# joesharratt1229/DT4Image_Restoration

Measured on AMD Instinct MI355X. Metric: pnp_admm_iterations_per_sec, higher is better.
Workload: dtype f32

## Files before the change

### dt4image_restoration_amd/_lib.py

```python
from __future__ import annotations

import ctypes as C
import os

_HERE = os.path.dirname(os.path.abspath(__file__))
LIB_PATH = os.environ.get("PNP_LIB_PATH") or os.path.join(_HERE, "csrc", "libpnpadmm.so")

PNP_FLAG_PROFILE = 1
PNP_FLAG_NO_DENOISER = 2
PNP_FLAG_KEEP_STAGES = 4
PNP_FLAG_BF16_CONVS = 8
PNP_FLAG_PROFILE_LAYERS = 16
PNP_SSIM_CLAMP_X = 1
PNP_RES_COLS = 6
PNP_RES_DELTA = 1
PNP_RES_DC = 2
RESIDUAL_COLUMNS = ("primal", "dx", "dz", "du", "delta", "dc")
PNP_MC_MAX_COILS = 32
PNP_MC_MAX_CG = 64
PNP_CC_MAX_COILS = 64
PNP_PW_MAX_COILS = 64
PNP_ESPIRIT_MAX_COILS = 16
PNP_ESPIRIT_MAX_KSIZE = 8
PNP_ESPIRIT_MAX_N = 512
# ... 78 lines not shown
    "pnp_restore": (C.c_int, [C.c_void_p, _vp, _fp, _fp, _fp, _fp, _vp]),
    "pnp_unet_read_stage": (C.c_int, [C.c_void_p, C.c_int, _fp, C.POINTER(C.c_int), C.POINTER(C.c_int),
                                      C.POINTER(C.c_int), _vp]),
    "pnp_profile_reset": (C.c_int, [C.c_void_p]),
    "pnp_profile_collect": (C.c_int, [C.c_void_p, C.POINTER(C.c_double), C.POINTER(C.c_int64)]),
    "pnp_profile_layers": (C.c_int, [C.c_void_p, C.POINTER(C.c_double), C.POINTER(C.c_int64)]),
    "pnp_conv_algorithms": (C.c_int, [C.c_void_p, C.POINTER(C.c_int32)]),
    "pnp_conv_schedules": (C.c_int, [C.c_void_p, C.POINTER(C.c_int32)]),
    "pnp_bf16_weight_terms": (C.c_int, [C.c_void_p]),
    "pnp_workspace_bytes": (C.c_size_t, [C.c_void_p]),
}

SIGNATURES_NCSENSE = {
    "pnp_nufft_forward_mc": (C.c_int, [C.c_void_p, _fp, _fp, C.c_int, C.c_int, C.c_int, _fp, _vp]),
    "pnp_nufft_adjoint_mc": (C.c_int, [C.c_void_p, _fp, _fp, _fp, C.c_int, C.c_int, C.c_int, _fp, _vp]),
    "pnp_set_kspace_ncsense": (C.c_int, [C.c_void_p, _fp, _fp, C.c_int, C.c_int, _fp, C.c_int, _vp]),
    "pnp_reset_ncsense": (C.c_int, [C.c_void_p, _fp, _fp, _fp, C.c_int, C.c_int, _fp, C.c_int, _fp, _fp, _fp, _vp]),
    "pnp_ncsense_coils": (C.c_int, [C.c_void_p]),
    "pnp_ncsense_cg_residual": (C.c_int, [C.c_void_p, _fp, _vp]),
    "pnp_ncsense_normal": (C.c_int, [C.c_void_p, _fp, _fp, _fp, _vp]),
    "pnp_acquire_ncsense": (C.c_int, [C.c_void_p, _fp, _fp, C.c_int, C.c_int, _fp, C.c_double, C.c_uint64, C.c_int, _fp, _fp, _fp, _vp]),
}

_lib = None


class PnPError(RuntimeError):
    pass


def load() -> C.CDLL:
    global _lib
    if _lib is not None:
        return _lib
    if not os.path.exists(LIB_PATH):
        raise PnPError(f"{LIB_PATH} not found: build it with `python -c 'import __graft_entry__ as g; g.build()'` "
                       f"or `make -C {os.path.dirname(LIB_PATH)}`; there is no CPU fallback")
    lib = C.CDLL(LIB_PATH)
    for name, (res, args) in {**SIGNATURES, **SIGNATURES_NCSENSE}.items():
        fn = getattr(lib, name)
        fn.restype = res
        fn.argtypes = args
    _lib = lib
    return lib


def check(rc: int, what: str) -> None:
    if rc != 0:
        msg = load().pnp_last_error()
        raise PnPError(f"{what} failed ({rc}): {msg.decode() if msg else '?'}")
```

### dt4image_restoration_amd/csrc/conv_kernels.hip

```cpp
#include "pnp_internal.h"
#include "conv_staging.h"
#include <cstring>
#include <cstdlib>

namespace pnp {



const LayerSpec kLayers[N_LAYERS] = {
    {2, 32, 3, 0, SRC_SIGMA, 0},    {32, 32, 3, 0, SRC_PLAIN, 0},   {32, 32, 3, 0, SRC_PLAIN, 0},
    {32, 64, 3, 1, SRC_POOL, 0},    {64, 64, 3, 1, SRC_PLAIN, 0},   {64, 64, 3, 1, SRC_PLAIN, 0},
    {64, 128, 3, 2, SRC_POOL, 0},   {128, 128, 3, 2, SRC_PLAIN, 0}, {128, 128, 3, 2, SRC_PLAIN, 0},
    {128, 256, 3, 3, SRC_POOL, 0},  {256, 256, 3, 3, SRC_PLAIN, 0}, {256, 256, 3, 3, SRC_PLAIN, 0},
    {256, 512, 3, 4, SRC_POOL, 0},  {512, 512, 3, 4, SRC_PLAIN, 0}, {512, 512, 3, 4, SRC_PLAIN, 0},
    {768, 256, 3, 3, SRC_UPCAT, 256}, {256, 256, 3, 3, SRC_PLAIN, 0}, {256, 256, 3, 3, SRC_PLAIN, 0},
    {384, 128, 3, 2, SRC_UPCAT, 128}, {128, 128, 3, 2, SRC_PLAIN, 0}, {128, 128, 3, 2, SRC_PLAIN, 0},
    {192, 64, 3, 1, SRC_UPCAT, 64},  {64, 64, 3, 1, SRC_PLAIN, 0},   {64, 64, 3, 1, SRC_PLAIN, 0},
    {96, 32, 3, 0, SRC_UPCAT, 32},   {32, 32, 3, 0, SRC_PLAIN, 0},   {32, 32, 3, 0, SRC_PLAIN, 0},
    {32, 1, 1, 0, SRC_PLAIN, 0},
};

ConvPlan conv3x3_plan(int N, int H, int W, int Cin, int Cout, bool bf16, int src_mode, bool allow_ws) {
    ConvPlan p{};
    p.tw = W >= 32 ? 32 : (W >= 16 ? 16 : 8);
// ... 623 lines not shown

bool conv3x3_pooled_output_ok(const ConvPlan& p) {
    return p.splitk == 1 && p.mt <= 2 && p.nt == 1 && p.wm == 4;
}

size_t conv3x3_partial_floats(const ConvPlan& p, int N, int H, int W, int Cout) {
    return (p.mt <= 2 && p.wn >= 2) ? (size_t)p.splitk * N * H * W * Cout : 0;
}

Tuning tuning_from_env() {
    Tuning t;
    if (const char* v = getenv("PNP_WINO_MIN_CIN")) t.wino_min_cin = atoi(v);
    if (const char* v = getenv("PNP_WINO_MIN_BLOCKS")) t.wino_min_blocks = atol(v);
    t.wino_big = getenv("PNP_WINO_BIG_GROUPS") != nullptr;
    t.wino_small = getenv("PNP_WINO_SMALL_GROUPS") != nullptr;
    t.no_wino = getenv("PNP_NO_WINOGRAD") != nullptr;
    if (const char* v = getenv("PNP_WINO_F4_MIN_CIN")) t.f4_min_cin = atoi(v);
    t.no_f4 = getenv("PNP_NO_WINO_F4") != nullptr;
    t.no_f4_phased = getenv("PNP_NO_WINO_F4_PHASED") != nullptr;
    t.no_f4_fused_last = getenv("PNP_NO_F4_FUSED_LAST") != nullptr;
    t.no_f4_fused_first = getenv("PNP_NO_F4_FUSED_FIRST") != nullptr;
    if (const char* v = getenv("PNP_WINO_F4_MT16")) t.f4_mt16 = atoi(v);
    if (const char* v = getenv("PNP_WINO_F4_CS")) t.f4_cs = atoi(v);
    if (const char* v = getenv("PNP_WINO_F4_ORDER")) t.f4_order = atoi(v) != 0;
    t.bf16_f32_acts = getenv("PNP_BF16_F32_ACTS") != nullptr;
    t.bf16_no_ws = getenv("PNP_BF16_NO_WS") != nullptr;
    t.bf16_w1 = getenv("PNP_BF16_W1") != nullptr;
    t.bf16_no_holdhi = getenv("PNP_BF16_NO_HOLDHI") != nullptr;
    if (const char* v = getenv("PNP_SLICE128_MIN_N")) t.slice128_min_n = atoi(v);
    if (const char* v = getenv("PNP_TV_NAIVE")) t.tv_naive = atoi(v) != 0;
    if (const char* v = getenv("PNP_HAAR_NAIVE")) t.haar_naive = atoi(v) != 0;
    if (const char* v = getenv("PNP_NCSENSE_COIL_BLOCK")) t.ncsense_block = atoi(v);
    if (const char* v = getenv("PNP_NCSENSE_NAIVE")) t.ncsense_naive = atoi(v) != 0 ? 1 : 0;
    return t;
}

hipError_t raise_lds_cap(const void* fn, int bytes, DeviceOnce& once) {
    int dev = 0;
    hipError_t e = hipGetDevice(&dev);
    if (e != hipSuccess) return e;
    const uint64_t bit = 1ull << (dev & 63);
    if (once.mask.load(std::memory_order_relaxed) & bit) return hipSuccess;
    e = hipFuncSetAttribute(fn, hipFuncAttributeMaxDynamicSharedMemorySize, bytes);
    if (e != hipSuccess) return e;
    once.mask.fetch_or(bit, std::memory_order_relaxed);
    return hipSuccess;
// ... 177 lines not shown
```

### dt4image_restoration_amd/csrc/pnp_capi.hip

```cpp
#include "../../include/pnpadmm.h"
#include "../../include/pnpadmm_ncsense.h"
#include "pnp_internal.h"
#include "denoiser_plan.h"
#include "nufft_plan.h"
#include "block_reduce.h"

#include <cmath>
#include <cstdarg>
#include <cstdio>
#include <cstring>
#include <cstdlib>
#include <initializer_list>
#include <new>
#include <string>
#include <vector>

using namespace pnp;

namespace {

thread_local std::string g_err;

int fail(int code, const char* fmt, ...) {
    char buf[512];
// ... 2061 lines not shown
    PNP_API_BEGIN
    if (!e || !algo28) return fail(PNP_ERR_INVALID, "pnp_conv_algorithms: null argument");
    if (e->cfg.flags & PNP_FLAG_NO_DENOISER) return fail(PNP_ERR_STATE, "pnp_conv_algorithms: handle has no denoiser");
    for (int i = 0; i < N_LAYERS; ++i) algo28[i] = e->dplan.family[i];
    return PNP_OK;
    PNP_API_END("pnp_conv_algorithms")
}

int pnp_conv_schedules(pnp_handle e, int32_t* sched28) {
    PNP_API_BEGIN
    if (!e || !sched28) return fail(PNP_ERR_INVALID, "pnp_conv_schedules: null argument");
    if (e->cfg.flags & PNP_FLAG_NO_DENOISER) return fail(PNP_ERR_STATE, "pnp_conv_schedules: handle has no denoiser");
    for (int i = 0; i < N_LAYERS; ++i) {
        const int at = e->dplan.launch_of[i];
        sched28[i] = 0;
        if (at < 0 || e->dplan.family[i] != FAM_WINO4) continue;
        const WinoPlan& w = e->dplan.launch[at].wino;
        sched28[i] = w.cs ? 4 : (w.mt == 16 ? 3 : (w.phased ? 2 : 1));
    }
    return PNP_OK;
    PNP_API_END("pnp_conv_schedules")
}

int pnp_profile_reset(pnp_handle e) {
    PNP_API_BEGIN
    if (!e) return fail(PNP_ERR_INVALID, "null handle");
    e->ev_used = 0;
    memset(e->cls_ms, 0, sizeof e->cls_ms); memset(e->cls_n, 0, sizeof e->cls_n);
    memset(e->layer_ms, 0, sizeof e->layer_ms); memset(e->layer_n, 0, sizeof e->layer_n);
    return PNP_OK;
    PNP_API_END("pnp_profile_reset")
}

int pnp_profile_collect(pnp_handle e, double* total_ms, int64_t* launches) {
    PNP_API_BEGIN
    if (!e) return fail(PNP_ERR_INVALID, "null handle");
    PNP_ON_DEVICE(e);
    for (size_t i = 0; i < e->ev_used; ++i) {
        float ms = 0.f;
        HIP_TRY(hipEventElapsedTime(&ms, e->events[i].a, e->events[i].b));
        const EventPair& p = e->events[i];
        e->cls_ms[p.cls] += ms; e->cls_n[p.cls] += p.count;
        if (p.layer >= 0) { e->layer_ms[p.layer] += ms; e->layer_n[p.layer] += 1; }
    }
    e->ev_used = 0;
    for (int i = 0; i < PNP_PROFILE_CLASSES; ++i) {
// ... 20 lines not shown
```

### dt4image_restoration_amd/csrc/pnp_internal.h

```cpp
#pragma once
#include <hip/hip_runtime.h>
#include <stdint.h>
#include <stddef.h>
#include <atomic>
#include <vector>

namespace pnp {

struct Tuning {
    int wino_min_cin = 32;
    long wino_min_blocks = 192;
    bool wino_big = false;
    bool wino_small = false;
    bool no_wino = false;
    int f4_min_cin = 32;
    bool no_f4 = false;
    bool no_f4_fused_first = false;
    bool no_f4_fused_last = false;
    bool no_f4_phased = false;
    int f4_mt16 = 0;
    bool bf16_no_ws = false;
    bool bf16_f32_acts = false;
    bool bf16_no_holdhi = false;
    bool bf16_w1 = false;
    int f4_cs = 1;
    int f4_order = 1;
    int slice128_min_n = 192;
    bool tv_naive = false;
    bool haar_naive = false;
    int ncsense_block = 0;
    int ncsense_naive = -1;
};
Tuning tuning_from_env();

struct DeviceOnce { std::atomic<uint64_t> mask{0}; };
hipError_t raise_lds_cap(const void* fn, int bytes, DeviceOnce& once);

enum SrcMode : int { SRC_PLAIN = 0, SRC_SIGMA = 1, SRC_POOL = 2, SRC_UPCAT = 3, SRC_FIRST = 4 };

struct LayerSpec {
    int cin, cout, ksize, level, src, cskip;
};
static constexpr int N_LAYERS = 28;
extern const LayerSpec kLayers[N_LAYERS];

struct ConvArgs {
    const float* src0;
    const float* src1;
// ... 31 lines not shown
    int tiles_x, tiles_y;
};
ConvPlan conv3x3_plan(int N, int H, int W, int Cin, int Cout, bool bf16 = false, int src_mode = SRC_PLAIN, bool allow_ws = true);
hipError_t launch_conv3x3_bf16ws(const ConvArgs& a, const ConvPlan& p, int src_mode, hipStream_t s);
size_t conv3x3_partial_floats(const ConvPlan& p, int N, int H, int W, int Cout);
bool conv3x3_pooled_output_ok(const ConvPlan& p);
bool conv3x3_tensor_fits(int N, int H, int W, int Cin, int Cout);
hipError_t launch_conv3x3(const ConvArgs& a, const ConvPlan& p, int src_mode, hipStream_t s);

size_t conv3x3_pack_floats(int cin, int cout);
void pack_conv3x3_weights(const float* oihw, int cin, int cout, int ck, float* dst);
size_t conv3x3_pack_floats_bf16(int cin, int cout, int terms);
void pack_conv3x3_weights_bf16(const float* oihw, int cin, int cout, int ck, int terms, float* dst);

struct WinoPlan {
    bool use;
    int algo;
    int tw, th, bn, wm, wn, ck, tiles_x, tiles_y;
    int stack;
    int mt;
    int phased;
    int cs;
    int order;
};
WinoPlan winograd_plan(int N, int H, int W, int Cin, int Cout, int src_mode, const Tuning& t, int Cskip = 0);
bool upsample_lines_regular(int H);
size_t winograd4_pack_floats(int cin, int cout);
void pack_winograd4_weights(const float* oihw, int cin, int cout, int ck, float* dst);
hipError_t launch_conv3x3_winograd4(const ConvArgs& a, const WinoPlan& p, int src_mode, hipStream_t s);
size_t winograd_pack_floats(int cin, int cout);
void pack_winograd_weights(const float* oihw, int cin, int cout, int ck, float* dst);
hipError_t launch_conv3x3_winograd(const ConvArgs& a, const WinoPlan& p, int src_mode, hipStream_t s);

hipError_t launch_conv_first(const float* ximg, const float2* z, const float2* u, const float* sigma,
                             const float* tact, const float* w, const float* bias, float* dst,
                             int N, int H, int W, hipStream_t s, bool dst_bf16 = false);
hipError_t launch_conv_last(const float* act, const float* ximg, const float2* z, const float2* u,
                            const float* tact, const float* w, const float* bias, float* out,
                            int N, int H, int W, hipStream_t s);
hipError_t launch_nhwc_to_nchw(const float* src, float* dst, int N, int C, int H, int W, hipStream_t s);

struct FftPlan {
    int h, w;
    float2* tw_h;
    float2* tw_w;
};
// ... 195 lines not shown
```

### dt4image_restoration_amd/csrc/winograd4_kernels.hip

```cpp
#include "pnp_internal.h"
#include "conv_staging.h"
#include <type_traits>

namespace pnp {

#ifdef PNP_STAMPS
#define W4_SLOTS 32
#define W4_WGS 1024
#define W4_N 16
__device__ unsigned long long g_w4_stamps[W4_SLOTS * W4_WGS * W4_N];
static int g_w4_slot = 0;
#define W4T() __builtin_amdgcn_s_memtime()
#endif

namespace {
constexpr double kA = 0.75, kB = 1.5;
constexpr float fA = 0.75f, fB = 1.5f, fA2 = 0.5625f, fB2 = 2.25f, fA3 = 0.421875f, fB3 = 3.375f;
constexpr float fK0 = 1.265625f;
constexpr float fK1 = 2.8125f;

__device__ __forceinline__ float4 f4add(float4 a, float4 b) { return make_float4(a.x + b.x, a.y + b.y, a.z + b.z, a.w + b.w); }
typedef float v2f __attribute__((ext_vector_type(2)));
typedef float f32x4 __attribute__((ext_vector_type(4)));

// ... 646 lines not shown
            if constexpr (FIRST) first_patch(c + 1);
            else park(c + 1, SPLIT ? 1 : 0);
        }
    }
#ifdef PNP_STAMPS
    st_loop1 = W4T();
    st_tmp = st_loop1;
#endif

    wino4_epilogue<TW, STK, MT, WN == 1 && MT == 32 && SRC == SRC_PLAIN>(a, acc, n, th, tg, cl, cb, tx0, ty0, STK ? (th == 0 ? live0 : live1) : true, smem);
#ifdef PNP_STAMPS
    {
        const int w = (int)blockIdx.x - (int)(gridDim.x / 2);
        if (tid == 0 && w >= 0 && w < W4_WGS && a.stamp_slot < W4_SLOTS) {
            unsigned long long* o = g_w4_stamps + ((size_t)a.stamp_slot * W4_WGS + w) * W4_N;
            const unsigned long long te = W4T();
            o[0] = 1; o[1] = st_setup - st_t0; o[2] = st_commit; o[3] = st_trans; o[4] = st_mfma; o[5] = st_loop1 - st_loop0;
            o[6] = te - st_tmp; o[7] = 0; o[8] = te - st_loop1; o[9] = te - st_t0; o[10] = (unsigned long long)nchunks;
        }
    }
#endif
}

template <int TW, bool STK>
__global__ __launch_bounds__(512, 2) void conv3x3_wino4p_kernel(const ConvArgs a) {
    constexpr int CK = 16, CKP = 16, PPP = 4, NT_ = 512, S = 4;
    constexpr int TC = TW / 4, TR = 32 / TC;
    constexpr int TH = 4 * TR;
    constexpr int SUBH = STK ? TH / 2 + 2 : 0;
    constexpr int PH = STK ? 2 * SUBH : TH + 2, PW = TW + 2;
    constexpr int NPIX = PH * PW, ITEMS = NPIX * PPP;
    constexpr int NIT = (ITEMS + NT_ - 1) / NT_;
    constexpr int PLSZ = ((NPIX * 4 + 15) / 16) * 16 + 4;
    constexpr int PATCH = 4 * PLSZ;
    constexpr int PF = 12, KEEP = 3;
    constexpr int PLANE = 32 * CKP;
    constexpr unsigned OOB = 0x80000000u;
    static_assert(!STK || TW == 16, "stacked slices: 16-wide tiles");
    static_assert((2 * PATCH + 36 * PLANE) * 4 <= 160 * 1024, "two patch copies + V in one CU's LDS");

    extern __shared__ __attribute__((aligned(16))) float smem[];
    float* const patch = smem;
    float* const V = smem + 2 * PATCH;
#ifdef PNP_STAMPS
    unsigned long long st_t0 = W4T(), st_setup = 0, st_loop0 = 0, st_commit = 0, st_trans = 0, st_mfma = 0, st_loop1 = 0, st_tmp = 0;
#endif
    const int tid = threadIdx.x, lane = tid & 63;
    const int wid = __builtin_amdgcn_readfirstlane(tid >> 6);
    const int grp = wid >> 2, cq = wid & 3;
    const int th = grp;
    const int tg = lane >> 4, cl = lane & 15;

    const int ny = a.Cout / 64;
    const int bid = blockIdx.x;
    const int ntl = a.tilesX * a.tilesY * (STK ? (a.N + 1) / 2 : a.N);
    int cby, bt;
    wino4_decode(bid, ny, ntl, a.order, cby, bt);
    if (bt >= ntl) return;
    const int tx0 = (bt % a.tilesX) * TW;
    bt /= a.tilesX;
    const int ty0 = (bt % a.tilesY) * TH;
    const int n = STK ? 2 * (bt / a.tilesY) : bt / a.tilesY;
    const int nsl = STK ? (n + 1 < a.N ? 2 : 1) : 1;
    const bool live0 = !(a.tact != nullptr && a.tact[n] > 0.5f);
    const bool live1 = STK && nsl == 2 && !(a.tact != nullptr && a.tact[n + 1] > 0.5f);
    if (!live0 && !live1) return;
    const int cb = cby * 4 + cq;
    const int nchunks = a.Cin / CK;
// ... 9 lines not shown
        const int sub = STK ? py / SUBH : 0;
        const int gy = STK ? py % SUBH - 1 : ty0 + py - 1, gx = tx0 + px - 1;
        voff[k] = (idx < ITEMS && sub < nsl && gy >= 0 && gy < a.H && gx >= 0 && gx < a.W)
                      ? (unsigned)((((sub * a.H + gy) * a.W + gx) * a.Cin + part * 4) * 4) : OOB;
    }
    const int ldst = (tid & 3) * PLSZ + (tid >> 2) * 4;
    float4 raw[NIT];
    auto issue = [&](int c) {
        const int soff = c * CK * 4;
#pragma unroll
        for (int k = 0; k < NIT; ++k)
            raw[k] = __builtin_bit_cast(float4, __builtin_amdgcn_raw_buffer_load_b128(rsrc0, voff[k], soff, 0));
    };
    auto park = [&](int c) {
        float* const dst = patch + (c & 1) * PATCH + ldst;
#pragma unroll
        for (int k = 0; k < NIT; ++k)
            if (tid + k * NT_ < ITEMS) *reinterpret_cast<float4*>(&dst[k * (NT_ / PPP) * 4]) = raw[k];
    };

    auto swz = [](int t16, int g) { return g ^ ((4 - (t16 >> 2)) & 3); };
    const int tgi = tid & 255;
    const int hc = tgi & 7, t16 = (tgi >> 3) & 15;
    const int tj = (wid >> 1) & 1;
    const int tq = 16 * grp + t16;
    const int trow = tq / TC;
    const int wrow = STK ? (trow / (TR / 2)) * SUBH + 4 * (trow % (TR / 2)) : 4 * trow;
    const int win = (hc >> 1) * PLSZ + (wrow * PW + 4 * (tq % TC)) * 4 + 2 * (hc & 1);
    const int vout = tq * CKP + 4 * swz(t16, hc >> 1) + 2 * (hc & 1);

    f32x4 acc[36];
#pragma unroll
    for (int k = 0; k < 36; ++k) acc[k] = f32x4{0.f, 0.f, 0.f, 0.f};

    const size_t stream = (size_t)nchunks * 36 * 64 + kW4Tail / S;
    const float4* const bptr = reinterpret_cast<const float4*>(a.wpack) + (size_t)cb * stream + lane;
    float4 bq[PF];
#pragma unroll
    for (int p = 0; p < KEEP; ++p) bq[p] = bptr[p * 64];
    const int aoff = (16 * th + cl) * CKP + 4 * swz(cl, tg);

    constexpr bool PARK_T = !STK;
    issue(0);
    park(0);
    if constexpr (!PARK_T) { if (grp == 1 && nchunks > 1) { issue(1); park(1); } }
#ifdef PNP_STAMPS
    st_setup = W4T();
    st_loop0 = st_setup;
#endif
    if (grp == 1) __syncthreads();
    for (int c = 0; c < nchunks; ++c) {
#ifdef PNP_STAMPS
        st_tmp = W4T();
#endif
        __syncthreads();
#ifdef PNP_STAMPS
        { const unsigned long long t = W4T(); st_commit += t - st_tmp; st_tmp = t; }
#endif
        if constexpr (PARK_T) { if (c + 1 < nchunks) issue(c + 1); }
        __builtin_amdgcn_s_setprio(3);
        {
            const float* const w = patch + (c & 1) * PATCH + win;
            if (tj == 0) wino4_input_transform<0, PW, 4, PLANE>(w, V + vout);
            else wino4_input_transform<1, PW, 4, PLANE>(w, V + vout);
        }
        __builtin_amdgcn_s_setprio(0);
        __builtin_amdgcn_sched_barrier(0);
        const float4* bp = bptr + (size_t)c * 36 * 64;
#pragma unroll
        for (int p = KEEP; p < PF; ++p) bq[p] = bp[p * 64];
        const int nx = c + 1 + grp;
        if constexpr (PARK_T) { if (c + 1 < nchunks) park(c + 1); }
        else { if (nx < nchunks) issue(nx); }
        __syncthreads();
#ifdef PNP_STAMPS
        { const unsigned long long t = W4T(); st_trans += t - st_tmp; st_tmp = t; }
#endif

        float4 ar[3];
        ar[0] = *reinterpret_cast<const float4*>(&V[aoff]);
        ar[1] = *reinterpret_cast<const float4*>(&V[PLANE + aoff]);
#pragma unroll
        for (int xi = 0; xi < 36; ++xi) {
            if (xi + 2 < 36) ar[(xi + 2) % 3] = *reinterpret_cast<const float4*>(&V[(xi + 2) * PLANE + aoff]);
            __builtin_amdgcn_sched_barrier(0);
            const float4 a0 = ar[xi % 3], b0 = bq[xi % PF];
            acc[xi] = __builtin_amdgcn_mfma_f32_16x16x4f32(a0.x, b0.x, acc[xi], 0, 0, 0);
            acc[xi] = __builtin_amdgcn_mfma_f32_16x16x4f32(a0.y, b0.y, acc[xi], 0, 0, 0);
            acc[xi] = __builtin_amdgcn_mfma_f32_16x16x4f32(a0.z, b0.z, acc[xi], 0, 0, 0);
            acc[xi] = __builtin_amdgcn_mfma_f32_16x16x4f32(a0.w, b0.w, acc[xi], 0, 0, 0);
            __builtin_amdgcn_sched_barrier(0);
#ifdef PNP_DIAG
            if ((a.diag & 4) && (xi & 1)) continue;
#endif
            if (xi + PF < 36 + KEEP) bq[xi % PF] = bp[(xi + PF) * 64];
        }
#ifdef PNP_STAMPS
        { const unsigned long long t = W4T(); st_mfma += t - st_tmp; }
#endif
        if constexpr (!PARK_T) { if (nx < nchunks) park(nx); }
    }
    if (grp == 0) __syncthreads();
#ifdef PNP_STAMPS
    st_loop1 = W4T();
    st_tmp = st_loop1;
#endif

    wino4_epilogue<TW, STK>(a, acc, n, th, tg, cl, cb, tx0, ty0, STK ? (th == 0 ? live0 : live1) : true);
#ifdef PNP_STAMPS
    {
        const int w = (int)blockIdx.x - (int)(gridDim.x / 2);
        if (tid == 0 && w >= 0 && w < W4_WGS && a.stamp_slot < W4_SLOTS) {
            unsigned long long* o = g_w4_stamps + ((size_t)a.stamp_slot * W4_WGS + w) * W4_N;
            const unsigned long long te = W4T();
            o[0] = 1; o[1] = st_setup - st_t0; o[2] = st_commit; o[3] = st_trans; o[4] = st_mfma; o[5] = st_loop1 - st_loop0;
            o[6] = te - st_tmp; o[7] = 0; o[8] = te - st_loop1; o[9] = te - st_t0; o[10] = (unsigned long long)nchunks;
        }
    }
#endif
}

template <int TW, int SRC>
__global__ __launch_bounds__(512, 2) void conv3x3_wino4c_kernel(const ConvArgs a) {
    constexpr int CK = 16, CKP = 16, PPP = 4, NT_ = 512, S = 4, MT = 16;
    constexpr bool UP2 = SRC == SRC_UPCAT;
    static_assert(SRC == SRC_PLAIN || SRC == SRC_UPCAT, "plain or upsample + concat source");
    constexpr int TC = TW / 4, TR = MT / TC;
    constexpr int TH = 4 * TR;
    constexpr int PH = TH + 2, PW = TW + 2;
    constexpr int NPIX = PH * PW, ITEMS = NPIX * PPP;
    constexpr int NIT = (ITEMS + NT_ - 1) / NT_;
    constexpr int PLSZ = ((NPIX * 4 + 15) / 16) * 16 + 4;
    constexpr int PATCH = 4 * PLSZ;
    constexpr int PF = 12, KEEP = 3;
    constexpr int PLANE = MT * CKP;
    constexpr int VSZ = 36 * PLANE;
    constexpr unsigned OOB = 0x80000000u;
    static_assert(NIT == 3 && ITEMS <= NIT * NT_, "three staging items per thread");
    constexpr int LP = CK;
// ... 212 lines not shown
        }
    }
#endif
}

template <int TW, int SRC>
static hipError_t launch_wino4c_inst(const ConvArgs& a, const WinoPlan& p, hipStream_t s) {
    constexpr int TC = TW / 4, TR = 16 / TC, TH = 4 * TR;
    constexpr int NPIX = (TH + 2) * (TW + 2);
    constexpr int PLSZ = ((NPIX * 4 + 15) / 16) * 16 + 4;
    constexpr size_t lowres_f = SRC == SRC_UPCAT ? (size_t)2 * (TH / 2 + 3) * (TW / 2 + 3) * 16 + 4 * (TH + 2 + TW + 2) : 0;
    constexpr size_t lds = ((size_t)2 * 4 * PLSZ + (size_t)2 * 36 * 16 * 16 + lowres_f) * sizeof(float);
    if (p.th != TH || p.tw != TW) return hipErrorInvalidValue;
    if (SRC == SRC_UPCAT && a.Cskip < 3 * 16) return hipErrorInvalidValue;
    auto kern = conv3x3_wino4c_kernel<TW, SRC>;
    static DeviceOnce cap;
    if (hipError_t e = raise_lds_cap((const void*)kern, (int)lds, cap); e != hipSuccess) return e;
    const int ntiles = p.tiles_x * p.tiles_y * a.N, ny = a.Cout / 128;
    dim3 grid((unsigned)(((ntiles + 7) / 8) * 8 * ny));
    hipLaunchKernelGGL(kern, grid, dim3(512), lds, s, a);
    return hipGetLastError();
}

template <int TW, bool STK>
static hipError_t launch_wino4p_inst(const ConvArgs& a, const WinoPlan& p, hipStream_t s) {
    constexpr int TC = TW / 4, TR = 32 / TC, TH = 4 * TR;
    constexpr int NPIX = (STK ? TH + 4 : TH + 2) * (TW + 2);
    constexpr int PLSZ = ((NPIX * 4 + 15) / 16) * 16 + 4;
    constexpr size_t lds = ((size_t)2 * 4 * PLSZ + (size_t)36 * 32 * 16) * sizeof(float);
    auto kern = conv3x3_wino4p_kernel<TW, STK>;
    static DeviceOnce cap;
    if (hipError_t e = raise_lds_cap((const void*)kern, (int)lds, cap); e != hipSuccess) return e;
    const int ntiles = p.tiles_x * p.tiles_y * (STK ? (a.N + 1) / 2 : a.N), ny = a.Cout / 64;
    dim3 grid((unsigned)(((ntiles + 7) / 8) * 8 * ny));
    hipLaunchKernelGGL(kern, grid, dim3(512), lds, s, a);
    return hipGetLastError();
}

template <int TW, int SRC, bool STK = false, int WN = 2, int MT = 32>
static hipError_t launch_wino4_inst(const ConvArgs& a, const WinoPlan& p, hipStream_t s) {
    constexpr int CK = 8 * WN, CKP = CK, CKQ = WN == 2 ? CK + 4 : CK + 2, TC = TW / 4, TR = MT / TC, TH = 4 * TR;
    constexpr size_t patch_f = (((size_t)(STK ? TH + 4 : TH + 2) * (TW + 2) * CKQ + 3) / 4) * 4;
    constexpr size_t lowres_f = SRC == SRC_UPCAT ? (size_t)(TH / 2 + 3) * (TW / 2 + 3) * CK + 4 * (TH + 2 + TW + 2) : 0;
    constexpr size_t first_f = SRC == SRC_FIRST ? (size_t)2 * (TH + 4) * (TW + 5) + 18 * 32 + 64 : 0;
    constexpr size_t lds = (patch_f + (size_t)36 * MT * CKP + lowres_f + first_f) * sizeof(float);
    static_assert(lds <= (WN == 2 && MT == 32 ? 160 : 80) * 1024, "one (8 waves) / two (4 waves) workgroups per CU");
    if (p.th != TH || p.tw != TW) return hipErrorInvalidValue;
    auto kern = conv3x3_wino4_kernel<TW, SRC, STK, WN, MT>;
    static DeviceOnce cap;
    if (hipError_t e = raise_lds_cap((const void*)kern, (int)lds, cap); e != hipSuccess) return e;
    const int ntiles = p.tiles_x * p.tiles_y * (STK ? (a.N + 1) / 2 : a.N), ny = a.Cout / (32 * WN);
    dim3 grid((unsigned)(((ntiles + 7) / 8) * 8 * ny));
    hipLaunchKernelGGL(kern, grid, dim3(8 * MT * WN), lds, s, a);
// ... 18 lines not shown
        if (p.tw == 16 && src_mode == SRC_FIRST) return launch_wino4_inst<16, SRC_FIRST, false, 1>(a, p, s);
        if (p.tw == 16 && src_mode == SRC_PLAIN) return launch_wino4_inst<16, SRC_PLAIN, false, 1>(a, p, s);
        if (p.tw == 16 && src_mode == SRC_UPCAT) return launch_wino4_inst<16, SRC_UPCAT, false, 1>(a, p, s);
        return hipErrorInvalidValue;
    }
    if (p.ck != 16) return hipErrorInvalidValue;
    if (p.cs) {
        if (p.bn != 128 || p.mt != 16 || p.stack) return hipErrorInvalidValue;
        if (p.tw == 32 && src_mode == SRC_PLAIN) return launch_wino4c_inst<32, SRC_PLAIN>(a, p, s);
        if (p.tw == 32 && src_mode == SRC_UPCAT) return launch_wino4c_inst<32, SRC_UPCAT>(a, p, s);
        if (p.tw == 16 && src_mode == SRC_PLAIN) return launch_wino4c_inst<16, SRC_PLAIN>(a, p, s);
        if (p.tw == 16 && src_mode == SRC_UPCAT) return launch_wino4c_inst<16, SRC_UPCAT>(a, p, s);
        return hipErrorInvalidValue;
    }
    if (p.mt == 16) {
        if (p.stack) return hipErrorInvalidValue;
        if (p.tw == 32 && src_mode == SRC_PLAIN) return launch_wino4_inst<32, SRC_PLAIN, false, 2, 16>(a, p, s);
        if (p.tw == 32 && src_mode == SRC_UPCAT) return launch_wino4_inst<32, SRC_UPCAT, false, 2, 16>(a, p, s);
        if (p.tw == 16 && src_mode == SRC_PLAIN) return launch_wino4_inst<16, SRC_PLAIN, false, 2, 16>(a, p, s);
        if (p.tw == 16 && src_mode == SRC_UPCAT) return launch_wino4_inst<16, SRC_UPCAT, false, 2, 16>(a, p, s);
        return hipErrorInvalidValue;
    }
    if (p.phased && src_mode == SRC_PLAIN) {
        if (p.tw == 32 && !p.stack) return launch_wino4p_inst<32, false>(a, p, s);
        if (p.tw == 16) {
            if (p.stack) return a.H == 16 && a.W == 16 ? launch_wino4p_inst<16, true>(a, p, s) : hipErrorInvalidValue;
            return launch_wino4p_inst<16, false>(a, p, s);
        }
        return hipErrorInvalidValue;
    }
    if (p.tw == 32) {
        if (src_mode == SRC_PLAIN) return launch_wino4_inst<32, SRC_PLAIN>(a, p, s);
        if (src_mode == SRC_UPCAT) return launch_wino4_inst<32, SRC_UPCAT>(a, p, s);
    } else if (p.tw == 16) {
        if (p.stack) return src_mode == SRC_PLAIN && a.H == 16 && a.W == 16 ? launch_wino4_inst<16, SRC_PLAIN, true>(a, p, s) : hipErrorInvalidValue;
        if (src_mode == SRC_PLAIN) return launch_wino4_inst<16, SRC_PLAIN>(a, p, s);
        if (src_mode == SRC_UPCAT) return launch_wino4_inst<16, SRC_UPCAT>(a, p, s);
    }
    return hipErrorInvalidValue;
}

}

#ifdef PNP_STAMPS
extern "C" int pnp_debug_stamps4_reset(void) { pnp::g_w4_slot = 0; return 0; }
extern "C" int pnp_debug_stamps4_read(unsigned long long* dst, int slots) {
    return (int)hipMemcpyFromSymbol(dst, HIP_SYMBOL(pnp::g_w4_stamps), (size_t)slots * W4_WGS * W4_N * sizeof(unsigned long long));
}
#endif
```

### dt4image_restoration_amd/csrc/winograd_kernels.hip

```cpp
#include "pnp_internal.h"
#include "conv_staging.h"
#include <cstdlib>

namespace pnp {

#ifdef PNP_STAMPS
#define PNP_STAMP_SLOTS 32
#define PNP_STAMP_WGS 1024
#define PNP_STAMP_N 112
__device__ unsigned long long g_wino_stamps[PNP_STAMP_SLOTS * PNP_STAMP_WGS * PNP_STAMP_N];
static int g_stamp_slot = 0;
#define STAMP() do { if (ns < PNP_STAMP_N) st[ns] = __builtin_amdgcn_s_memtime(); ++ns; } while (0)
#else
#define STAMP() do { } while (0)
#endif

size_t winograd_pack_floats(int cin, int cout) { return (size_t)(cout / 32) * ((size_t)(cin / 8) * 16 * 256 + 2 * 4 * 256); }

void pack_winograd_weights(const float* oihw, int cin, int cout, int ck, float* dst) {
    static const double G[4][3] = {{1, 0, 0}, {0.5, 0.5, 0.5}, {0.5, -0.5, 0.5}, {0, 0, 1}};
    std::vector<float> U((size_t)cout * cin * 16);
    for (int co = 0; co < cout; ++co)
        for (int ci = 0; ci < cin; ++ci) {
            const float* g = oihw + ((size_t)co * cin + ci) * 9;
// ... 45 lines not shown
            f.mt = 32;
            const bool mt16 = t.f4_mt16 == 0 ? (src_mode == SRC_UPCAT || Cin <= 64) : (t.f4_mt16 == 1 ? false : (t.f4_mt16 == 2 ? src_mode == SRC_UPCAT : true));
            if (f.bn == 64 && mt16 && (f.tw == 32 ? H >= 8 : H >= 16)) {
                f.mt = 16;
                f.th = f.tw == 32 ? 8 : 16;
                f.tiles_y = (H + f.th - 1) / f.th;
                f.stack = 0;
            }
            f.phased = (f.mt == 32 && f.bn == 64 && src_mode == SRC_PLAIN && !t.no_f4_phased) ? 1 : 0;
            const bool cs_can = f.bn == 64 && Cout % 128 == 0 && (src_mode == SRC_PLAIN || (Cskip % 16 == 0 && Cskip >= 48));
            const int cs_th = f.tw == 32 ? 8 : 16;
            const long cs_blocks = (long)f.tiles_x * ((H + cs_th - 1) / cs_th) * N * (Cout / 128);
            const bool cs_rule = src_mode == SRC_UPCAT && cs_blocks >= kCsMinBlocks;
            if (cs_can && cs_blocks >= t.wino_min_blocks && (t.f4_cs == 2 || (t.f4_cs == 1 && t.f4_mt16 == 0 && !t.no_f4_phased && cs_rule))) {
                f.cs = 1;
                f.bn = 128;
                f.mt = 16;
                f.th = cs_th;
                f.tiles_y = (H + f.th - 1) / f.th;
                f.stack = 0;
                f.phased = 0;
            }
            const long blocks = (long)f.tiles_x * f.tiles_y * (f.stack ? (N + 1) / 2 : N) * (Cout / f.bn);
            f.use = blocks >= t.wino_min_blocks;
            if (f.use) return f;
        }
    }
    p.tw = W >= 32 ? 32 : (W >= 16 ? 16 : 8);
    const bool big = t.wino_big;
    if (Cout % 128 == 0 && !t.wino_small) { p.wm = 1; p.wn = 4; p.ck = 32; }
    else if (Cout % 64 == 0) { if (big) { p.wm = 2; p.wn = 2; } else { p.wm = 1; p.wn = 2; } p.ck = 16; }
    else { if (big) { p.wm = 4; p.wn = 1; } else { p.wm = 2; p.wn = 1; } p.ck = 8; }
    const int tc = p.tw / 2, tr = 32 / tc;
    p.th = p.wm * 2 * tr;
    p.bn = p.wn * 32;
    p.tiles_x = (W + p.tw - 1) / p.tw;
    p.tiles_y = (H + p.th - 1) / p.th;
    const long blocks = (long)p.tiles_x * p.tiles_y * N * (Cout / p.bn);
    p.use = blocks >= t.wino_min_blocks;
    return p;
}

template <int TW, int WM, int WN, int CK, int SRC>
__global__ __launch_bounds__(WM * WN * 128, 2) void conv3x3_winograd_kernel(const ConvArgs a) {
    constexpr int GW = WM * WN;
    constexpr int NT_ = GW * 128;
// ... 378 lines not shown
```

### dt4image_restoration_amd/engine.py

```python
from __future__ import annotations

import ctypes as C
from typing import Dict, Mapping, Optional, Tuple

import numpy as np
import torch

from . import _lib
from .weights import flatten_state_dict

RESIDUAL_COLUMNS = _lib.RESIDUAL_COLUMNS


def _ptr(t: Optional[torch.Tensor]) -> Optional[int]:
    return None if t is None else t.data_ptr()


_episode_counter = 0


def _next_episode() -> int:
    global _episode_counter
    _episode_counter += 1
    return _episode_counter
# ... 647 lines not shown
            raise ValueError("not a snapshot of this engine")
        _lib.check(self.lib.pnp_restore(self._h, snap.data_ptr(), x.data_ptr(), z.data_ptr(), u.data_ptr(), _ptr(t_state),
                                        self._stream()), "pnp_restore")

    def read_stage(self, which: int) -> torch.Tensor:
        c, hh, ww = C.c_int(), C.c_int(), C.c_int()
        _lib.check(self.lib.pnp_unet_read_stage(self._h, which, None, C.byref(c), C.byref(hh), C.byref(ww), self._stream()),
                   "pnp_unet_read_stage")
        out = torch.empty((self.n, c.value, hh.value, ww.value), dtype=torch.float32, device=self.device)
        _lib.check(self.lib.pnp_unet_read_stage(self._h, which, out.data_ptr(), None, None, None, self._stream()),
                   "pnp_unet_read_stage")
        return out

    def conv_algorithms(self):
        out = (C.c_int32 * _lib.N_LAYERS)()
        _lib.check(self.lib.pnp_conv_algorithms(self._h, out), "pnp_conv_algorithms")
        return list(out)

    def conv_schedules(self):
        out = (C.c_int32 * _lib.N_LAYERS)()
        _lib.check(self.lib.pnp_conv_schedules(self._h, out), "pnp_conv_schedules")
        return list(out)

    def bf16_weight_terms(self) -> int:
        return int(self.lib.pnp_bf16_weight_terms(self._h))

    def profile_reset(self) -> None:
        _lib.check(self.lib.pnp_profile_reset(self._h), "pnp_profile_reset")

    def profile_collect(self) -> Dict[str, Dict[str, float]]:
        ms = (C.c_double * _lib.PROFILE_CLASSES)()
        cnt = (C.c_int64 * _lib.PROFILE_CLASSES)()
        _lib.check(self.lib.pnp_profile_collect(self._h, ms, cnt), "pnp_profile_collect")
        lms = (C.c_double * _lib.N_LAYERS)()
        lcnt = (C.c_int64 * _lib.N_LAYERS)()
        _lib.check(self.lib.pnp_profile_layers(self._h, lms, lcnt), "pnp_profile_layers")
        out = {name: {"ms": ms[i], "launches": int(cnt[i])} for i, name in enumerate(_lib.PROFILE_CLASS_NAMES)}
        out["layers"] = {"ms": list(lms), "launches": [int(v) for v in lcnt]}
        return out
```

Baseline: 133.0.

## Split Winograd-4 phased kernel frequencies across wave groups with accumulator exchange

Adds an FS variant of the phased Winograd F(4,3) conv kernel. Each wave group now handles half of the 36 transform frequencies for all 32 tiles, instead of all frequencies for half the tiles. Each thread then prefetches only its half of the weight stream (PF 12 to 6), and the partial accumulators are swapped through LDS after the main loop so the existing epilogue still works. By default it is enabled only for stacked 16x16 layers with at least 256 blocks. The aim is to halve per-wave weight-load traffic and register pressure, at the cost of an extra LDS exchange and two barriers.

```diff
diff --git a/dt4image_restoration_amd/_lib.py b/dt4image_restoration_amd/_lib.py
--- a/dt4image_restoration_amd/_lib.py
+++ b/dt4image_restoration_amd/_lib.py
@@ -124,6 +124,10 @@
     "pnp_acquire_ncsense": (C.c_int, [C.c_void_p, _fp, _fp, C.c_int, C.c_int, _fp, C.c_double, C.c_uint64, C.c_int, _fp, _fp, _fp, _vp]),
 }
 
+SIGNATURES_PLAN = {
+    "pnp_conv_fsplit": (C.c_int, [C.c_void_p, C.POINTER(C.c_int32)]),
+}
+
 _lib = None
 
 
@@ -139,7 +143,7 @@
         raise PnPError(f"{LIB_PATH} not found: build it with `python -c 'import __graft_entry__ as g; g.build()'` "
                        f"or `make -C {os.path.dirname(LIB_PATH)}`; there is no CPU fallback")
     lib = C.CDLL(LIB_PATH)
-    for name, (res, args) in {**SIGNATURES, **SIGNATURES_NCSENSE}.items():
+    for name, (res, args) in {**SIGNATURES, **SIGNATURES_NCSENSE, **SIGNATURES_PLAN}.items():
         fn = getattr(lib, name)
         fn.restype = res
         fn.argtypes = args
diff --git a/dt4image_restoration_amd/csrc/conv_kernels.hip b/dt4image_restoration_amd/csrc/conv_kernels.hip
--- a/dt4image_restoration_amd/csrc/conv_kernels.hip
+++ b/dt4image_restoration_amd/csrc/conv_kernels.hip
@@ -669,6 +669,7 @@
     t.no_f4_fused_first = getenv("PNP_NO_F4_FUSED_FIRST") != nullptr;
     if (const char* v = getenv("PNP_WINO_F4_MT16")) t.f4_mt16 = atoi(v);
     if (const char* v = getenv("PNP_WINO_F4_CS")) t.f4_cs = atoi(v);
+    if (const char* v = getenv("PNP_WINO_F4_FSPLIT")) t.f4_fsplit = atoi(v);
     if (const char* v = getenv("PNP_WINO_F4_ORDER")) t.f4_order = atoi(v) != 0;
     t.bf16_f32_acts = getenv("PNP_BF16_F32_ACTS") != nullptr;
     t.bf16_no_ws = getenv("PNP_BF16_NO_WS") != nullptr;
diff --git a/dt4image_restoration_amd/csrc/pnp_capi.hip b/dt4image_restoration_amd/csrc/pnp_capi.hip
--- a/dt4image_restoration_amd/csrc/pnp_capi.hip
+++ b/dt4image_restoration_amd/csrc/pnp_capi.hip
@@ -1,5 +1,6 @@
 #include "../../include/pnpadmm.h"
 #include "../../include/pnpadmm_ncsense.h"
+#include "../../include/pnpadmm_plan.h"
 #include "pnp_internal.h"
 #include "denoiser_plan.h"
 #include "nufft_plan.h"
@@ -2107,6 +2108,18 @@
     PNP_API_END("pnp_conv_schedules")
 }
 
+int pnp_conv_fsplit(pnp_handle e, int32_t* flags28) {
+    PNP_API_BEGIN
+    if (!e || !flags28) return fail(PNP_ERR_INVALID, "pnp_conv_fsplit: null argument");
+    if (e->cfg.flags & PNP_FLAG_NO_DENOISER) return fail(PNP_ERR_STATE, "pnp_conv_fsplit: handle has no denoiser");
+    for (int i = 0; i < N_LAYERS; ++i) {
+        const int at = e->dplan.launch_of[i];
+        flags28[i] = (at >= 0 && e->dplan.family[i] == FAM_WINO4 && e->dplan.launch[at].wino.phased && e->dplan.launch[at].wino.fsplit) ? 1 : 0;
+    }
+    return PNP_OK;
+    PNP_API_END("pnp_conv_fsplit")
+}
+
 int pnp_profile_reset(pnp_handle e) {
     PNP_API_BEGIN
     if (!e) return fail(PNP_ERR_INVALID, "null handle");
diff --git a/dt4image_restoration_amd/csrc/pnp_internal.h b/dt4image_restoration_amd/csrc/pnp_internal.h
--- a/dt4image_restoration_amd/csrc/pnp_internal.h
+++ b/dt4image_restoration_amd/csrc/pnp_internal.h
@@ -24,6 +24,7 @@
     bool bf16_no_holdhi = false;
     bool bf16_w1 = false;
     int f4_cs = 1;
+    int f4_fsplit = 1;
     int f4_order = 1;
     int slice128_min_n = 192;
     bool tv_naive = false;
@@ -101,6 +102,7 @@
     int phased;
     int cs;
     int order;
+    int fsplit;
 };
 WinoPlan winograd_plan(int N, int H, int W, int Cin, int Cout, int src_mode, const Tuning& t, int Cskip = 0);
 bool upsample_lines_regular(int H);
diff --git a/dt4image_restoration_amd/csrc/winograd4_kernels.hip b/dt4image_restoration_amd/csrc/winograd4_kernels.hip
--- a/dt4image_restoration_amd/csrc/winograd4_kernels.hip
+++ b/dt4image_restoration_amd/csrc/winograd4_kernels.hip
@@ -692,7 +692,7 @@
 #endif
 }
 
-template <int TW, bool STK>
+template <int TW, bool STK, bool FS = false>
 __global__ __launch_bounds__(512, 2) void conv3x3_wino4p_kernel(const ConvArgs a) {
     constexpr int CK = 16, CKP = 16, PPP = 4, NT_ = 512, S = 4;
     constexpr int TC = TW / 4, TR = 32 / TC;
@@ -703,17 +703,18 @@
     constexpr int NIT = (ITEMS + NT_ - 1) / NT_;
     constexpr int PLSZ = ((NPIX * 4 + 15) / 16) * 16 + 4;
     constexpr int PATCH = 4 * PLSZ;
-    constexpr int PF = 12, KEEP = 3;
+    constexpr int PF = FS ? 6 : 12, KEEP = 3;
     constexpr int PLANE = 32 * CKP;
     constexpr unsigned OOB = 0x80000000u;
     static_assert(!STK || TW == 16, "stacked slices: 16-wide tiles");
     static_assert((2 * PATCH + 36 * PLANE) * 4 <= 160 * 1024, "two patch copies + V in one CU's LDS");
+    static_assert(!FS || (2 * PATCH + 36 * PLANE) * 4 >= 8 * 18 * 64 * 16, "FS: the accumulator exchange fits the patch + V space in one round");
 
     extern __shared__ __attribute__((aligned(16))) float smem[];
     float* const patch = smem;
     float* const V = smem + 2 * PATCH;
 #ifdef PNP_STAMPS
-    unsigned long long st_t0 = W4T(), st_setup = 0, st_loop0 = 0, st_commit = 0, st_trans = 0, st_mfma = 0, st_loop1 = 0, st_tmp = 0;
+    unsigned long long st_t0 = W4T(), st_setup = 0, st_loop0 = 0, st_commit = 0, st_trans = 0, st_mfma = 0, st_loop1 = 0, st_tmp = 0, st_xchg = 0;
 #endif
     const int tid = threadIdx.x, lane = tid & 63;
     const int wid = __builtin_amdgcn_readfirstlane(tid >> 6);
@@ -769,8 +770,8 @@
     auto swz = [](int t16, int g) { return g ^ ((4 - (t16 >> 2)) & 3); };
     const int tgi = tid & 255;
     const int hc = tgi & 7, t16 = (tgi >> 3) & 15;
-    const int tj = (wid >> 1) & 1;
-    const int tq = 16 * grp + t16;
+    const int tj = FS ? grp : (wid >> 1) & 1;
+    const int tq = FS ? tgi >> 3 : 16 * grp + t16;
     const int trow = tq / TC;
     const int wrow = STK ? (trow / (TR / 2)) * SUBH + 4 * (trow % (TR / 2)) : 4 * trow;
     const int win = (hc >> 1) * PLSZ + (wrow * PW + 4 * (tq % TC)) * 4 + 2 * (hc & 1);
@@ -781,11 +782,12 @@
     for (int k = 0; k < 36; ++k) acc[k] = f32x4{0.f, 0.f, 0.f, 0.f};
 
     const size_t stream = (size_t)nchunks * 36 * 64 + kW4Tail / S;
-    const float4* const bptr = reinterpret_cast<const float4*>(a.wpack) + (size_t)cb * stream + lane;
+    auto fxi = [](int k) { return 36 * (k / 18) + 6 * ((k % 18) / 3) + k % 3; };
+    const float4* const bptr = reinterpret_cast<const float4*>(a.wpack) + (size_t)cb * stream + lane + (FS ? 3 * grp * 64 : 0);
     float4 bq[PF];
 #pragma unroll
     for (int p = 0; p < KEEP; ++p) bq[p] = bptr[p * 64];
-    const int aoff = (16 * th + cl) * CKP + 4 * swz(cl, tg);
+    const int aoff = FS ? cl * CKP + 4 * swz(cl, tg) + 3 * grp * PLANE : (16 * th + cl) * CKP + 4 * swz(cl, tg);
 
     constexpr bool PARK_T = !STK;
     issue(0);
@@ -815,7 +817,7 @@
         __builtin_amdgcn_sched_barrier(0);
         const float4* bp = bptr + (size_t)c * 36 * 64;
 #pragma unroll
-        for (int p = KEEP; p < PF; ++p) bq[p] = bp[p * 64];
+        for (int p = KEEP; p < PF; ++p) bq[p] = bp[(FS ? fxi(p) : p) * 64];
         const int nx = c + 1 + grp;
         if constexpr (PARK_T) { if (c + 1 < nchunks) park(c + 1); }
         else { if (nx < nchunks) issue(nx); }
@@ -824,6 +826,36 @@
         { const unsigned long long t = W4T(); st_trans += t - st_tmp; st_tmp = t; }
 #endif
 
+        if constexpr (FS) {
+            float4 ar[3][2];
+#pragma unroll
+            for (int k = 0; k < 2; ++k)
+#pragma unroll
+                for (int m = 0; m < 2; ++m) ar[k][m] = *reinterpret_cast<const float4*>(&V[fxi(k) * PLANE + aoff + m * 16 * CKP]);
+#pragma unroll
+            for (int k = 0; k < 18; ++k) {
+                if (k + 2 < 18) {
+#pragma unroll
+                    for (int m = 0; m < 2; ++m) ar[(k + 2) % 3][m] = *reinterpret_cast<const float4*>(&V[fxi(k + 2) * PLANE + aoff + m * 16 * CKP]);
+                }
+                __builtin_amdgcn_sched_barrier(0);
+                const float4 a0 = ar[k % 3][0], a1 = ar[k % 3][1], b0 = bq[k % PF];
+                const int i0 = 6 * (k / 3) + k % 3, i1 = i0 + 3;
+                acc[i0] = __builtin_amdgcn_mfma_f32_16x16x4f32(a0.x, b0.x, acc[i0], 0, 0, 0);
+                acc[i1] = __builtin_amdgcn_mfma_f32_16x16x4f32(a1.x, b0.x, acc[i1], 0, 0, 0);
+                acc[i0] = __builtin_amdgcn_mfma_f32_16x16x4f32(a0.y, b0.y, acc[i0], 0, 0, 0);
+                acc[i1] = __builtin_amdgcn_mfma_f32_16x16x4f32(a1.y, b0.y, acc[i1], 0, 0, 0);
+                acc[i0] = __builtin_amdgcn_mfma_f32_16x16x4f32(a0.z, b0.z, acc[i0], 0, 0, 0);
+                acc[i1] = __builtin_amdgcn_mfma_f32_16x16x4f32(a1.z, b0.z, acc[i1], 0, 0, 0);
+                acc[i0] = __builtin_amdgcn_mfma_f32_16x16x4f32(a0.w, b0.w, acc[i0], 0, 0, 0);
+                acc[i1] = __builtin_amdgcn_mfma_f32_16x16x4f32(a1.w, b0.w, acc[i1], 0, 0, 0);
+                __builtin_amdgcn_sched_barrier(0);
+#ifdef PNP_DIAG
+                if ((a.diag & 4) && (k & 1)) continue;
+#endif
+                if (k + PF < 18 + KEEP) bq[k % PF] = bp[fxi(k + PF) * 64];
+            }
+        } else {
         float4 ar[3];
         ar[0] = *reinterpret_cast<const float4*>(&V[aoff]);
         ar[1] = *reinterpret_cast<const float4*>(&V[PLANE + aoff]);
@@ -842,6 +874,7 @@
 #endif
             if (xi + PF < 36 + KEEP) bq[xi % PF] = bp[(xi + PF) * 64];
         }
+        }
 #ifdef PNP_STAMPS
         { const unsigned long long t = W4T(); st_mfma += t - st_tmp; }
 #endif
@@ -852,6 +885,30 @@
     st_loop1 = W4T();
     st_tmp = st_loop1;
 #endif
+    if constexpr (FS) {
+        __syncthreads();
+        float4* const xw = reinterpret_cast<float4*>(smem) + wid * (18 * 64) + lane;
+        const float4* const xr = reinterpret_cast<const float4*>(smem) + (wid ^ 4) * (18 * 64) + lane;
+        if (grp == 0) {
+#pragma unroll
+            for (int k = 0; k < 18; ++k) xw[k * 64] = __builtin_bit_cast(float4, acc[6 * (k / 3) + 3 + k % 3]);
+        } else {
+#pragma unroll
+            for (int k = 0; k < 18; ++k) xw[k * 64] = __builtin_bit_cast(float4, acc[6 * (k / 3) + k % 3]);
+        }
+        __syncthreads();
+        if (grp == 0) {
+#pragma unroll
+            for (int k = 0; k < 18; ++k) acc[6 * (k / 3) + 3 + k % 3] = __builtin_bit_cast(f32x4, xr[k * 64]);
+        } else {
+#pragma unroll
+            for (int k = 0; k < 18; ++k) acc[6 * (k / 3) + k % 3] = __builtin_bit_cast(f32x4, xr[k * 64]);
+        }
+#ifdef PNP_STAMPS
+        st_tmp = W4T();
+        st_xchg = st_tmp - st_loop1;
+#endif
+    }
 
     wino4_epilogue<TW, STK>(a, acc, n, th, tg, cl, cb, tx0, ty0, STK ? (th == 0 ? live0 : live1) : true);
 #ifdef PNP_STAMPS
@@ -861,7 +918,7 @@
             unsigned long long* o = g_w4_stamps + ((size_t)a.stamp_slot * W4_WGS + w) * W4_N;
             const unsigned long long te = W4T();
             o[0] = 1; o[1] = st_setup - st_t0; o[2] = st_commit; o[3] = st_trans; o[4] = st_mfma; o[5] = st_loop1 - st_loop0;
-            o[6] = te - st_tmp; o[7] = 0; o[8] = te - st_loop1; o[9] = te - st_t0; o[10] = (unsigned long long)nchunks;
+            o[6] = te - st_tmp; o[7] = 0; o[8] = te - st_loop1; o[9] = te - st_t0; o[10] = (unsigned long long)nchunks; o[11] = st_xchg;
         }
     }
 #endif
@@ -1120,13 +1177,13 @@
     return hipGetLastError();
 }
 
-template <int TW, bool STK>
+template <int TW, bool STK, bool FS>
 static hipError_t launch_wino4p_inst(const ConvArgs& a, const WinoPlan& p, hipStream_t s) {
     constexpr int TC = TW / 4, TR = 32 / TC, TH = 4 * TR;
     constexpr int NPIX = (STK ? TH + 4 : TH + 2) * (TW + 2);
     constexpr int PLSZ = ((NPIX * 4 + 15) / 16) * 16 + 4;
     constexpr size_t lds = ((size_t)2 * 4 * PLSZ + (size_t)36 * 32 * 16) * sizeof(float);
-    auto kern = conv3x3_wino4p_kernel<TW, STK>;
+    auto kern = conv3x3_wino4p_kernel<TW, STK, FS>;
     static DeviceOnce cap;
     if (hipError_t e = raise_lds_cap((const void*)kern, (int)lds, cap); e != hipSuccess) return e;
     const int ntiles = p.tiles_x * p.tiles_y * (STK ? (a.N + 1) / 2 : a.N), ny = a.Cout / 64;
@@ -1191,10 +1248,13 @@
         return hipErrorInvalidValue;
     }
     if (p.phased && src_mode == SRC_PLAIN) {
-        if (p.tw == 32 && !p.stack) return launch_wino4p_inst<32, false>(a, p, s);
+        if (p.tw == 32 && !p.stack) return p.fsplit ? launch_wino4p_inst<32, false, true>(a, p, s) : launch_wino4p_inst<32, false, false>(a, p, s);
         if (p.tw == 16) {
-            if (p.stack) return a.H == 16 && a.W == 16 ? launch_wino4p_inst<16, true>(a, p, s) : hipErrorInvalidValue;
-            return launch_wino4p_inst<16, false>(a, p, s);
+            if (p.stack) {
+                if (a.H != 16 || a.W != 16) return hipErrorInvalidValue;
+                return p.fsplit ? launch_wino4p_inst<16, true, true>(a, p, s) : launch_wino4p_inst<16, true, false>(a, p, s);
+            }
+            return p.fsplit ? launch_wino4p_inst<16, false, true>(a, p, s) : launch_wino4p_inst<16, false, false>(a, p, s);
         }
         return hipErrorInvalidValue;
     }
diff --git a/dt4image_restoration_amd/csrc/winograd_kernels.hip b/dt4image_restoration_amd/csrc/winograd_kernels.hip
--- a/dt4image_restoration_amd/csrc/winograd_kernels.hip
+++ b/dt4image_restoration_amd/csrc/winograd_kernels.hip
@@ -91,6 +91,8 @@
                 f.phased = 0;
             }
             const long blocks = (long)f.tiles_x * f.tiles_y * (f.stack ? (N + 1) / 2 : N) * (Cout / f.bn);
+            const bool fs_rule = f.stack && blocks >= 256;
+            f.fsplit = (f.phased && (t.f4_fsplit == 2 || (t.f4_fsplit == 1 && t.f4_mt16 == 0 && t.f4_cs == 1 && t.f4_order == 1 && fs_rule))) ? 1 : 0;
             f.use = blocks >= t.wino_min_blocks;
             if (f.use) return f;
         }
diff --git a/dt4image_restoration_amd/engine.py b/dt4image_restoration_amd/engine.py
--- a/dt4image_restoration_amd/engine.py
+++ b/dt4image_restoration_amd/engine.py
@@ -693,6 +693,11 @@
         _lib.check(self.lib.pnp_conv_schedules(self._h, out), "pnp_conv_schedules")
         return list(out)
 
+    def conv_fsplit(self):
+        out = (C.c_int32 * _lib.N_LAYERS)()
+        _lib.check(self.lib.pnp_conv_fsplit(self._h, out), "pnp_conv_fsplit")
+        return list(out)
+
     def bf16_weight_terms(self) -> int:
         return int(self.lib.pnp_bf16_weight_terms(self._h))
 
diff --git a/include/pnpadmm_plan.h b/include/pnpadmm_plan.h
--- /dev/null
+++ b/include/pnpadmm_plan.h
@@ -0,0 +1,16 @@
+#ifndef PNPADMM_PLAN_H
+#define PNPADMM_PLAN_H
+
+#include "pnpadmm.h"
+
+#ifdef __cplusplus
+extern "C" {
+#endif
+
+int pnp_conv_fsplit(pnp_handle h, int32_t* flags28);
+
+#ifdef __cplusplus
+}
+#endif
+
+#endif
```

New measurement: 133.3, median of 6. About the same (+0.2%).
